# unpause-live/SwiftVideo

Measured on AMD Instinct MI355X. Metric: Gpix/s + achieved HBM GB/s, 1080p NV12→BGRA+scale+4-layer composite, 1/2/4/8 GPU, higher is better.
Workload: dtype f32; 1 GPU; pipeline: 4 x 1080p NV12 -> BGRA (BT.601 int) + bilinear scale to 720p + 4-layer alpha composite, one launch per batch; frames_per_launch_per_gpu=256, kernel=tick_bgra_stream, full=False

## Files before the change

swiftvideo_amd/csrc/chipvideo.cpp:

```cpp
#include "../../include/chipvideo.h"

#include <hip/hip_runtime.h>
#include <hip/hiprtc.h>

#include <algorithm>
#include <atomic>
#include <cctype>
#include <cstdarg>
#include <cmath>
#include <cstdio>
#include <cstring>
#include <map>
#include <memory>
#include <mutex>
#include <string>
#include <vector>

#include "device_types.h"
#include "switches.h"
#include "geom_cache.h"
#include "rebind.h"
#include "lanczos_planar.h"

namespace chv {
const char *bgra_wave_build_flags();
const char *yuv_wave_build_flags();
const char *bgra_stream_build_flags();
const char *yuv_stream_build_flags();
const char *lanczos_build_flags();
hipError_t launch_tick_general(int target_format, const DTick *ticks_host, const DLayer *layers_host, const DTick *ticks, const DLayer *layers,
                               int n_ticks, int maxW, int maxH, hipStream_t stream);
hipError_t launch_selftest(float *out_f, const float *in_f, uint8_t *out_c, const float *num,
                           const float *den, float *out_q, int n, hipStream_t stream);
hipError_t launch_selftest_pack(const int *b, const int *g, const int *r, uint32_t *out, int n, hipStream_t stream);
hipError_t launch_selftest_pack_codes(const float *in, uint32_t *out, int n, hipStream_t stream);
hipError_t launch_selftest_matrices(int dir, int csc, uint32_t *out, uint32_t *mism, hipStream_t stream);
const char *fast_path_name(int path);
bool wave_layers_by_value(int target_format, const DTick *tick_host, const DLayer *layers_host);
bool fast_path_is_wave(int path);
bool fast_path_by_value(int path);
int split_stream_prefix(const DTick *ticks, const DLayer *layers, int n_ticks);
int fast_path_stream_bgra();
int select_tail_path(int target_format, const DTick *ticks, const DLayer *layers, int n_ticks);
int select_fast_path(int target_format, const DTick *ticks, const DLayer *layers, int n_ticks, bool transient = false);
hipError_t launch_tick_fast(int path, const DTick *ticks_host, const DLayer *layers_host,
                            const DTick *ticks, const DLayer *layers, int n_ticks,
                            int maxW, int maxH, hipStream_t stream, GeomCache *tables);
hipError_t launch_snd_s16i(int16_t *out, const int16_t *const *in, int count, int n, const float *gain, const float *fade, hipStream_t stream);
hipError_t launch_me_fullsearch(const DPlane &out, const DPlane &ref, const DPlane &cur, const int32_t *block, const int32_t *window, const int32_t *image,
                                const float *cost256, hipStream_t stream);
hipError_t launch_lanczos(const DPlane &dst, const DPlane &src, const int32_t *fx, const float *wx,
                          int tx, const int32_t *fy, const float *wy, int ty, hipStream_t stream,
                          const DPlane *batch, int n_batch, int stride_x, int first_x, int stride_y);
}

using namespace chv;

static void g_detail_set(const char *msg);

static int parse_switch(const char *name, const char *value, int *out) {
    const std::string n = name ? name : "", v = value ? value : "";
    if (n == "CHV_FORCE_GENERAL") { *out = v == "1" ? 1 : 0; return 0; }
    if (n == "CHV_BGRA_PATH") { *out = v == "wave" ? 1 : v == "tiled" ? 2 : v == "stream" ? 3 : 0; return 1; }
    if (n == "CHV_WAVE_ROWS") { *out = v == "8" ? 8 : v == "16" ? 16 : 0; return 2; }
    if (n == "CHV_TILE_ROWS") { *out = v == "16" ? 16 : v == "32" ? 32 : 0; return 3; }
    if (n == "CHV_SAME_GEOM") { *out = v == "0" ? 0 : 1; return 4; }
    if (n == "CHV_DESC") { *out = v == "host" ? 1 : v == "device" ? 2 : 0; return 5; }
    if (n == "CHV_STREAM") { *out = v == "0" ? 0 : 1; return 6; }
    if (n == "CHV_YUV_STREAM") { *out = v == "0" ? 0 : (v == "force" || v == "2") ? 2 : 1; return 7; }
    if (n == "CHV_WAVE_DMA") { *out = v == "0" ? 0 : 1; return 8; }
    if (n == "CHV_PASS_FUSE") { *out = v == "0" ? 0 : 1; return 9; }
    if (n == "CHV_GEOM_CACHE") { *out = v == "0" ? 0 : v == "eager" ? 2 : 1; return 10; }
    if (n == "CHV_STREAM_ROWS") { const int r = atoi(v.c_str()); *out = (r >= 1 && r <= 4096) ? r : 0; return 11; }
    if (n == "CHV_STREAM_OPAQUE") { *out = v == "0" ? 0 : 1; return 12; }
    if (n == "CHV_REBIND") { *out = v == "scatter" ? 1 : v == "copy" ? 2 : 0; return 13; }
    return -1;
}
static void store_switch(Switches &s, int which, int val) {
    std::atomic<int> *slots[14] = { &s.force_general, &s.bgra_path, &s.wave_rows, &s.tile_rows, &s.same_geom, &s.desc_host, &s.stream, &s.yuv_stream, &s.wave_dma,
                                    &s.pass_fuse, &s.geom_cache, &s.stream_rows, &s.stream_opaque, &s.rebind };
    slots[which]->store(val, std::memory_order_relaxed);
}
Switches &chv::switches() {
    static Switches s;
    static std::once_flag once;
    std::call_once(once, [] {
        static const char *const names[14] = { "CHV_FORCE_GENERAL", "CHV_BGRA_PATH", "CHV_WAVE_ROWS", "CHV_TILE_ROWS", "CHV_SAME_GEOM", "CHV_DESC", "CHV_STREAM", "CHV_YUV_STREAM",
                                               "CHV_WAVE_DMA", "CHV_PASS_FUSE", "CHV_GEOM_CACHE", "CHV_STREAM_ROWS", "CHV_STREAM_OPAQUE", "CHV_REBIND" };
        for (const char *n : names) {
            const char *v = getenv(n);
            int val = 0, which = v ? parse_switch(n, v, &val) : -1;
            if (which >= 0) store_switch(s, which, val);
        }
    });
    return s;
}
static std::atomic<RebindLauncher> g_rebind_launcher{nullptr};
void chv::register_rebind_launcher(RebindLauncher fn) { g_rebind_launcher.store(fn, std::memory_order_release); }
static std::atomic<LanczosPlanarLauncher> g_lanczos_planar_launcher{nullptr};
void chv::register_lanczos_planar_launcher(LanczosPlanarLauncher fn) { g_lanczos_planar_launcher.store(fn, std::memory_order_release); }
DebugCounters &chv::debug_counters() {
    static DebugCounters c;
    return c;
}
extern "C" int chv_debug_set_switch(const char *name, const char *value) {
    int val = 0;
    Switches &s = switches();
    const int which = parse_switch(name, value, &val);
    if (which < 0) { g_detail_set("unknown switch"); return CHV_ERR_INVALID_VALUE; }
    if (!value || !*value) val = (which == 4 || which == 6 || which == 7 || which == 8 || which == 9 || which == 10 || which == 12) ? 1 : 0;
    store_switch(s, which, val);
    return CHV_OK;
}
extern "C" int chv_debug_get_counter(const char *name, unsigned long long *value) {
    static const char *const names[] = { "geom_store_patched", "geom_store_batch_hits", "geom_store_builds", "geom_store_bytes", "geom_store_tables" };
    if (!name || !value) { g_detail_set("null argument"); return CHV_ERR_INVALID_VALUE; }
    for (int i = 0; i < 5; i++)
        if (!strcmp(name, names[i])) { *value = (unsigned long long)geom_store_counter(i); return CHV_OK; }
    if (!strcmp(name, "stream_opaque_launches")) { *value = debug_counters().stream_opaque_launches.load(std::memory_order_relaxed); return CHV_OK; }
    g_detail_set("unknown counter");
    return CHV_ERR_INVALID_VALUE;
}
extern "C" const char *chv_build_flags(void) {
    static const std::string flags = std::string("arch=" CHV_ARCH ";hipcc=" CHV_HIPCC_VERSION ";clang=") + std::to_string(__clang_major__) + "." + std::to_string(__clang_minor__) +
                                     ";fp_contract=off;" + bgra_wave_build_flags() + ";" + yuv_wave_build_flags() + ";" + bgra_stream_build_flags() + ";" +
                                     yuv_stream_build_flags() + ";" + lanczos_build_flags() +
                                     (g_rebind_launcher.load(std::memory_order_acquire) ? ";batch_rebind:scatter=1" : ";batch_rebind:scatter=0");
    return flags.c_str();
}

static thread_local std::string g_detail;
static void g_detail_set(const char *msg) { g_detail = msg; }

static int fail(int code, const char *fmt, ...) __attribute__((format(printf, 2, 3)));
static int fail(int code, const char *fmt, ...) {
    char buf[512];
    va_list ap;
    va_start(ap, fmt);
    vsnprintf(buf, sizeof buf, fmt, ap);
    va_end(ap);
    g_detail = buf;
    return code;
}

static int hip_fail(hipError_t e, const char *what) {
    int code = CHV_ERR_UNKNOWN;
    switch (e) {
    case hipErrorOutOfMemory: code = CHV_ERR_OUT_OF_MEMORY; break;
    case hipErrorInvalidValue: code = CHV_ERR_INVALID_VALUE; break;
    case hipErrorInvalidDevice: code = CHV_ERR_INVALID_DEVICE; break;
    case hipErrorNoDevice: code = CHV_ERR_DEVICE_NOT_AVAILABLE; break;
    case hipErrorInvalidContext: code = CHV_ERR_INVALID_CONTEXT; break;
    case hipErrorNotSupported: code = CHV_ERR_NOT_IMPLEMENTED; break;
    default: break;
    }
    return fail(code, "%s: %s (%d)", what, hipGetErrorString(e), (int)e);
}
#define HIP_TRY(expr)                                         \
    do {                                                      \
        hipError_t _e = (expr);                               \
        if (_e != hipSuccess) return hip_fail(_e, #expr);     \
    } while (0)

extern "C" const char *chv_error_string(int s) {
    switch (s) {
    case CHV_OK: return "success";
    case CHV_ERR_INVALID_VALUE: return "invalidValue";
    case CHV_ERR_OUT_OF_MEMORY: return "outOfMemory";
    case CHV_ERR_INVALID_CONTEXT: return "invalidContext";
    case CHV_ERR_BAD_TARGET: return "badTarget";
    case CHV_ERR_BAD_INPUT: return "badInputData";
    case CHV_ERR_NOT_IMPLEMENTED: return "notImplemented";
    case CHV_ERR_KERNEL_NOT_FOUND: return "computeKernelNotFound";
    case CHV_ERR_DEVICE_NOT_AVAILABLE: return "deviceNotAvailable";
    case CHV_ERR_INVALID_DEVICE: return "invalidDevice";
    case CHV_ERR_INVALID_OPERATION: return "invalidOperation";
    case CHV_ERR_BAD_CONTEXT_STATE: return "badContextState";
    case CHV_ERR_INVALID_PLATFORM: return "invalidPlatform";
    default: return "unknownError";
    }
}
extern "C" const char *chv_last_error_detail(void) { return g_detail.c_str(); }
extern "C" int chv_version(void) { return CHV_VERSION; }

struct KernelName { const char *name; int id; };
static const KernelName kNames[] = {
    { "img_nv12_nv12", CHV_K_IMG_NV12_NV12 },   { "img_bgra_nv12", CHV_K_IMG_BGRA_NV12 },
    { "img_rgba_nv12", CHV_K_IMG_RGBA_NV12 },   { "img_bgra_bgra", CHV_K_IMG_BGRA_BGRA },
    { "img_y420p_y420p", CHV_K_IMG_Y420P_Y420P }, { "img_y420p_nv12", CHV_K_IMG_Y420P_NV12 },
    { "img_clear_nv12", CHV_K_IMG_CLEAR_NV12 }, { "img_clear_yuvs", CHV_K_IMG_CLEAR_YUVS },
    { "img_clear_bgra", CHV_K_IMG_CLEAR_BGRA }, { "img_clear_rgba", CHV_K_IMG_CLEAR_BGRA },
    { "img_rgba_y420p", CHV_K_IMG_RGBA_Y420P }, { "img_bgra_y420p", CHV_K_IMG_BGRA_Y420P },
    { "img_clear_y420p", CHV_K_IMG_CLEAR_Y420P },
    { "img_nv12_bgra", CHV_K_IMG_NV12_BGRA },   { "img_y420p_bgra", CHV_K_IMG_Y420P_BGRA },
    { "img_bgra_bgra_tx", CHV_K_IMG_BGRA_BGRA_TX }, { "img_rgba_bgra_tx", CHV_K_IMG_RGBA_BGRA_TX },
    { "img_rgba_bgra", CHV_K_IMG_RGBA_BGRA_TX },
    { "img_bgra_nv12_int", CHV_K_IMG_BGRA_NV12_INT }, { "img_rgba_nv12_int", CHV_K_IMG_RGBA_NV12_INT },
    { "img_bgra_y420p_int", CHV_K_IMG_BGRA_Y420P_INT }, { "img_rgba_y420p_int", CHV_K_IMG_RGBA_Y420P_INT },
    { "snd_s16i_s16i", CHV_K_SND_S16I_S16I }, { "me_fullsearch", CHV_K_ME_FULLSEARCH },
};

extern "C" int chv_kernel_from_string(const char *name, int *kernel) {
// ... 2058 lines not shown
```

swiftvideo_amd/csrc/kernels_stream.hip.cpp:

```cpp
#include "kernels_stream_body.hip.inc"
#include "stream_select.h"

namespace chv {

hipError_t launch_bgra_stream_opaque(const DTick *ticks_host, const DLayer *layers_host, const DTick *ticks, const DLayer *layers, int n_ticks, bool planar, dim3 grid,
                                     size_t lds, int strips_x, int chunks_y, int rows, hipStream_t stream);

template <int NL, bool PL, bool ABS>
__global__ __launch_bounds__(64 * ST_WAVES, CHV_STREAM_WAVES) void tick_bgra_stream(const DTick *__restrict__ ticks, const DLayer *__restrict__ layers, int n_ticks,
                                                                          int strips_x, int chunks_y, int rows_per_chunk) {
    stream_body<NL, false, PL, ABS>(ticks, layers, n_ticks, strips_x, chunks_y, rows_per_chunk);
}

template <int NL, bool PL, bool ABS>
__global__ __launch_bounds__(64 * ST_WAVES, CHV_STREAM_WAVES) void tick_bgra_stream_one(const StreamOne<NL> a, int strips_x, int chunks_y, int rows_per_chunk) {
    stream_body<NL, true, PL, ABS>(&a.t, a.l, 1, strips_x, chunks_y, rows_per_chunk);
}

static bool stream_plane_ok(const DPlane &p) {
    return (((uintptr_t)p.ptr) & 15) == 0 && (p.pitch & 15) == 0 && ((p.w * p.comps) & 15) == 0 && p.w * p.comps >= 16 && p.h >= 1;
}

#define CHV_STR2(x) #x
#define CHV_STR(x) CHV_STR2(x)
const char *bgra_stream_build_flags() { return "tick_bgra_stream:abl=" CHV_STR(CHV_ST_ABL) ",strips_per_block=" CHV_STR(CHV_STREAM_BLOCK) ",rounds=" CHV_STR(CHV_STREAM_ROUNDS); }

bool bgra_stream_eligible(const DTick *ticks, const DLayer *layers, int n_ticks) {
    if (n_ticks < 1 || !switches().stream.load(std::memory_order_relaxed)) return false;
    const int nl = ticks[0].n_layers;
    if (nl < 1 || nl > 4) return false;
    for (int i = 0; i < n_ticks; i++) {
        const DTick &T = ticks[i];
        if (T.n_layers != nl || !T.clear_first) return false;
        if ((((uintptr_t)T.dst.pl[0].ptr) & 3) != 0 || (T.dst.pl[0].pitch & 3) != 0) return false;
        for (int l = 0; l < nl; l++) {
            const DLayer &Y = layers[T.first_layer + l];
            const int kind0 = layers[ticks[0].first_layer].kind;
            if ((kind0 != LK_BGRA_FROM_NV12 && kind0 != LK_BGRA_FROM_Y420P) || Y.kind != kind0) return false;
            const bool planar = kind0 == LK_BGRA_FROM_Y420P;
            const int need = LF_AXIS_ALIGNED | LF_BOUNDED | LF_NO_FILL | (l ? LF_SAME_GEOM : 0);
            if ((Y.flags & need) != need) return false;
            const float op = Y.u[U_OPACITY];
            if (!(op >= 0.f && op <= 1.f)) return false;
            if (!stream_plane_ok(Y.src.pl[0]) || !stream_plane_ok(Y.src.pl[1])) return false;
            if (Y.src.pl[0].h > 32767 || Y.src.pl[1].h > 16383) return false;
            if (Y.src.pl[1].comps != (planar ? 1 : 2) || Y.src.pl[0].comps != 1) return false;
            if (planar) {
                const DPlane &cu = Y.src.pl[1], &cv = Y.src.pl[2];
                if (!stream_plane_ok(cv) || cv.comps != 1 || cv.w != cu.w || cv.h != cu.h || cv.pitch != cu.pitch) return false;
            }
            if (l == 0) {
                const double kx = 2.0 * (double)Y.u[U_TRANSFORM + 0] * (double)Y.u[U_TEXTURE + 0], ky = 2.0 * (double)Y.u[U_TRANSFORM + 5] * (double)Y.u[U_TEXTURE + 5];
                if (!(kx > 0.0) || !(ky > 0.0)) return false;
                const double sx = kx * Y.src.pl[0].w / (double)T.W;
                if (!(63.0 * sx + 2.0 + 15.0 + 1.0 <= 128.0)) return false;
                if (planar && !(63.0 * (kx * Y.src.pl[1].w / (double)T.W) + 2.0 + 15.0 + 1.0 <= (double)ST_CPP)) return false;
                const double sy = ky * Y.src.pl[0].h / (double)T.H;
                if (!std::isfinite(sy) || sy > 4.0) return false;
            }
        }
    }
    return true;
}

hipError_t launch_bgra_stream(const DTick *ticks_host, const DLayer *layers_host, const DTick *ticks, const DLayer *layers, int n_ticks, int maxW, int maxH, hipStream_t stream) {
    const int nl = ticks_host[0].n_layers;
    const int strips_x = (maxW + 63) / 64;
    const long want = 1024L * CHV_STREAM_WAVES * CHV_STREAM_ROUNDS;
    const long chunks = std::max<long>(1, want / std::max<long>(1, (long)n_ticks * strips_x));
    const long wave_rows = (long)n_ticks * strips_x * maxH;
    const long rows_small = std::min<long>(CHV_STREAM_SMALL_ROWS_MAX, std::max<long>(CHV_STREAM_MIN_ROWS, (wave_rows + CHV_STREAM_SMALL_WAVES - 1) / CHV_STREAM_SMALL_WAVES));
    int rows = (int)std::max<long>(rows_small, (maxH + chunks - 1) / chunks);
    if (CHV_STREAM_ROWS_FIXED > 0) rows = CHV_STREAM_ROWS_FIXED;
    if (const int forced = switches().stream_rows.load(std::memory_order_relaxed)) rows = forced;
    rows = std::max(1, std::min(rows, maxH));
    const int chunks_y = (maxH + rows - 1) / rows;
    const long total = (long)n_ticks * chunks_y * ((strips_x + ST_WAVES - 1) / ST_WAVES);
    dim3 grid((unsigned)(((total + 7) / 8) * 8));
    const bool planar = layers_host[ticks_host[0].first_layer].kind == LK_BGRA_FROM_Y420P;
    const size_t layer_bytes = planar ? (size_t)st_layer_bytes<1, true>() : (size_t)st_layer_bytes<1, false>();
    const size_t lds = (size_t)ST_WAVES * ((size_t)nl * layer_bytes + ST_TAB * (sizeof(uint4) + sizeof(uint32_t)));
    bool absorb = CHV_STREAM_ABSORB != 0;
    for (int i = 0; i < n_ticks && absorb; i++)
        for (int l = 0; l < nl; l++) absorb = absorb && csc_absorbable(layers_host[ticks_host[i].first_layer + l].csc);
    if (absorb && stream_opaque_bottom(ticks_host, layers_host, n_ticks, switches().stream_opaque.load(std::memory_order_relaxed))) {
        const hipError_t err = launch_bgra_stream_opaque(ticks_host, layers_host, ticks, layers, n_ticks, planar, grid, lds, strips_x, chunks_y, rows, stream);
        if (err == hipSuccess) debug_counters().stream_opaque_launches.fetch_add(1, std::memory_order_relaxed);
        return err;
    }
    if (!ticks) {
        if (n_ticks != 1 || !layers_host) return hipErrorInvalidValue;
        auto go = [&](auto tag) {
            constexpr int NL = decltype(tag)::value;
            StreamOne<NL> a;
            a.t = ticks_host[0];
            a.t.first_layer = 0;
            for (int l = 0; l < NL; l++) a.l[l] = layers_host[ticks_host[0].first_layer + l];
            auto fire = [&](auto pl, auto ab) {
                hipLaunchKernelGGL((tick_bgra_stream_one<NL, decltype(pl)::value, decltype(ab)::value>), grid, dim3(64 * ST_WAVES), lds, stream, a, strips_x, chunks_y, rows);
            };
            if (planar) { if (absorb) fire(std::true_type{}, std::true_type{}); else fire(std::true_type{}, std::false_type{}); }
            else { if (absorb) fire(std::false_type{}, std::true_type{}); else fire(std::false_type{}, std::false_type{}); }
        };
        switch (nl) {
        case 1: go(std::integral_constant<int, 1>{}); break;
        case 2: go(std::integral_constant<int, 2>{}); break;
        case 3: go(std::integral_constant<int, 3>{}); break;
        default: go(std::integral_constant<int, 4>{}); break;
        }
        return hipGetLastError();
    }
#define CHV_ST_GO2(N, P, A) hipLaunchKernelGGL((tick_bgra_stream<N, P, A>), grid, dim3(64 * ST_WAVES), lds, stream, ticks, layers, n_ticks, strips_x, chunks_y, rows)
#define CHV_ST_GO(N) do { if (planar) { if (absorb) CHV_ST_GO2(N, true, true); else CHV_ST_GO2(N, true, false); } \
                          else { if (absorb) CHV_ST_GO2(N, false, true); else CHV_ST_GO2(N, false, false); } } while (0)
    switch (nl) {
    case 1: CHV_ST_GO(1); break;
    case 2: CHV_ST_GO(2); break;
    case 3: CHV_ST_GO(3); break;
    default: CHV_ST_GO(4); break;
    }
#undef CHV_ST_GO
#undef CHV_ST_GO2
    return hipGetLastError();
}

}
```

swiftvideo_amd/csrc/kernels_stream_body.hip.inc:

```
#pragma once
#include "wave_common.hip.h"
#include "switches.h"

#include <algorithm>
#include <type_traits>
#include <cmath>

#pragma clang fp contract(off)

namespace chv {

#ifndef CHV_ST_ABL
#define CHV_ST_ABL 0
#endif
#ifndef CHV_STREAM_ABSORB
#define CHV_STREAM_ABSORB 1
#endif
#ifndef CHV_STREAM_PMIX
#define CHV_STREAM_PMIX 1
#endif
#ifndef CHV_STREAM_ROWS_FIXED
#define CHV_STREAM_ROWS_FIXED 0
#endif
#ifndef CHV_STREAM_SMALL_WAVES
#define CHV_STREAM_SMALL_WAVES 4800
#endif
#ifndef CHV_STREAM_SMALL_ROWS_MAX
#define CHV_STREAM_SMALL_ROWS_MAX 12
#endif
#ifndef CHV_STREAM_MIN_ROWS
#define CHV_STREAM_MIN_ROWS 4
#endif
#ifndef CHV_STREAM_ROUNDS
#define CHV_STREAM_ROUNDS 12
#endif
#ifndef CHV_STREAM_WAVES
#define CHV_STREAM_WAVES 6
#endif

constexpr float kRintBias = 8388608.0f;
constexpr int ST_PITCH = 128;
constexpr int ST_YROWS = 8, ST_CROWS = 4;
constexpr int ST_YL = 4 * ST_PITCH, ST_CL = 2 * ST_PITCH;
constexpr int ST_CPP = 96, ST_CLP = 2 * ST_CPP;
template <int NL, bool PL> constexpr int st_layer_bytes() { return ST_PITCH * ST_YROWS + (PL ? 2 * 2 * ST_CLP : ST_PITCH * ST_CROWS); }
constexpr int ST_TAB = 32;
#ifndef CHV_STREAM_BLOCK
#define CHV_STREAM_BLOCK 4
#endif
constexpr int ST_WAVES = CHV_STREAM_BLOCK;


CHV_DEV void st_dma(const uint8_t *p, bool active, uint32_t m0) {
    if (active && !(CHV_ST_ABL & 1))
        asm volatile("s_mov_b32 m0, %0\n\ts_nop 0\n\tglobal_load_lds_dwordx4 %1, off" :: "s"(m0), "v"(p) : "memory");
}

CHV_DEV void st_store(uint8_t *row, uint32_t off, uint32_t v) {
    asm volatile("global_store_dword %0, %1, %2" :: "v"(off), "v"(v), "s"(row) : "memory");
}

struct StTaps { uint32_t y00, y10, y01, y11, u00, u10, u01, u11, v00, v10, v01, v11; };
template <int LO, int LC, int LV>
CHV_DEV void st_taps_read(StTaps &t, uint32_t aY00, uint32_t aY10, uint32_t aY01, uint32_t aY11, uint32_t aC00, uint32_t aC10, uint32_t aC01, uint32_t aC11) {
    asm volatile("ds_read_u8 %0, %12 offset:%20\n\tds_read_u8 %1, %13 offset:%20\n\tds_read_u8 %2, %14 offset:%20\n\tds_read_u8 %3, %15 offset:%20\n\t"
                 "ds_read_u8 %4, %16 offset:%21\n\tds_read_u8 %5, %17 offset:%21\n\tds_read_u8 %6, %18 offset:%21\n\tds_read_u8 %7, %19 offset:%21\n\t"
                 "ds_read_u8 %8, %16 offset:%22\n\tds_read_u8 %9, %17 offset:%22\n\tds_read_u8 %10, %18 offset:%22\n\tds_read_u8 %11, %19 offset:%22"
                 : "=&v"(t.y00), "=&v"(t.y10), "=&v"(t.y01), "=&v"(t.y11), "=&v"(t.u00), "=&v"(t.u10), "=&v"(t.u01), "=&v"(t.u11),
                   "=&v"(t.v00), "=&v"(t.v10), "=&v"(t.v01), "=&v"(t.v11)
                 : "v"(aY00), "v"(aY10), "v"(aY01), "v"(aY11), "v"(aC00), "v"(aC10), "v"(aC01), "v"(aC11), "n"(LO), "n"(LC), "n"(LV));
}
template <int YOUNGER>
CHV_DEV void st_taps_wait(StTaps &t) {
    asm volatile("s_waitcnt lgkmcnt(%12)"
                 : "+v"(t.y00), "+v"(t.y10), "+v"(t.y01), "+v"(t.y11), "+v"(t.u00), "+v"(t.u10), "+v"(t.u01), "+v"(t.u11), "+v"(t.v00), "+v"(t.v10), "+v"(t.v01), "+v"(t.v11)
                 : "n"(YOUNGER));
}

template <int NL, bool ONE, bool PL, bool ABS, bool OPQ = false>
CHV_DEV void stream_body(const DTick *__restrict__ ticks, const DLayer *__restrict__ layers, int n_ticks, int strips_x, int chunks_y, int rows_per_chunk) {
    extern __shared__ __attribute__((aligned(16))) uint8_t lds_all[];
    constexpr int LBYTES = st_layer_bytes<NL, PL>();
    constexpr int CPITCH = PL ? ST_CPP : ST_PITCH, CLB = PL ? ST_CLP : ST_CL;
    constexpr int VOFF = PL ? 2 * NL * ST_CLP : 1;
    constexpr int WBYTES = NL * LBYTES + ST_TAB * (int)(sizeof(uint4) + sizeof(uint32_t));
    const int wave = __builtin_amdgcn_readfirstlane((int)threadIdx.x >> 6);
    uint8_t *lds = lds_all + wave * WBYTES;
    uint4 *rowtab = (uint4 *)(lds + NL * LBYTES);
    uint32_t *rowpos = (uint32_t *)(rowtab + ST_TAB);
    const uint32_t lds0 = (uint32_t)(size_t)lds;
    static_assert(!OPQ || (NL >= 2 && ABS && CHV_STREAM_PMIX), "the opaque-bottom form: two layers or more, absorbed matrices, binary16 blend inputs");
    const int lane = threadIdx.x & 63;
    const int groups_x = (strips_x + ST_WAVES - 1) / ST_WAVES;
    const int total = n_ticks * chunks_y * groups_x;
    const int b = blockIdx.x, per_xcd = (total + 7) >> 3;
    const int idx = (b & 7) * per_xcd + (b >> 3);
    if ((b >> 3) >= per_xcd || idx >= total) return;
    const int tick = idx / (chunks_y * groups_x), rem = idx - tick * (chunks_y * groups_x);
    const int chunk = rem / groups_x, strip = (rem - chunk * groups_x) * ST_WAVES + wave;
    if (strip >= strips_x) return;
    const DTick &T = ticks[ONE ? 0 : tick];
    const DLayer *L = layers + (ONE ? 0 : T.first_layer);
    const int x0 = strip * 64, y0 = chunk * rows_per_chunk;
    if (x0 >= T.W || y0 >= T.H) return;
    const int nrows = min(rows_per_chunk, T.H - y0);
    const DPlane D = T.dst.pl[0];
    const float sx = (float)T.W, sy = (float)T.H;
    const float *U = L[0].u;
    const DPlane SY = L[0].src.pl[0], SC = L[0].src.pl[1];

    const int x = x0 + lane, xe = min(x, T.W - 1);
    const float nx = ((float)xe / sx) * 2.f - 1.f;
    const float t3 = U[U_TRANSFORM + 15];
    const float t0 = nx * U[U_TRANSFORM + 0] + U[U_TRANSFORM + 3];
    const float b0 = nx * U[U_BORDER + 0] + U[U_BORDER + 3];
    const float u = t0 * U[U_TEXTURE + 0] + t3 * U[U_TEXTURE + 3];
    const int cfl = ((b0 >= 0.f && b0 <= 1.f) ? AX_BORDER : 0) | ((t0 >= 0.f && t0 <= 1.f) ? AX_TX : 0) | ((u >= 0.f && u <= 1.f) ? AX_UV : 0);
    int cy, cc;
    float cya, cca;
    lin_axis_raw(u, SY.w, cy, cya); lin_axis_raw(u, SC.w, cc, cca);
    const int cy_first = __builtin_amdgcn_readfirstlane(cy), cc_first = __builtin_amdgcn_readfirstlane(cc);
    const int ycol0 = min(max(cy_first, 0), SY.w - 1) & ~15;
    constexpr int BPC = PL ? 1 : 2;
    const int ccol0 = (min(max(cc_first, 0), SC.w - 1) * BPC) & ~15;
    const int oy0 = min(max(min(max(cy, 0), SY.w - 1) - ycol0, 0), ST_PITCH - 1), oy1 = min(max(min(max(cy + 1, 0), SY.w - 1) - ycol0, 0), ST_PITCH - 1);
    const int oc0 = min(max(min(max(cc, 0), SC.w - 1) * BPC - ccol0, 0), CPITCH - BPC), oc1 = min(max(min(max(cc + 1, 0), SC.w - 1) * BPC - ccol0, 0), CPITCH - BPC);
    int oc0v = oc0, oc1v = oc1;
    asm("" : "+v"(oc0v), "+v"(oc1v));
    const float iya = (1.0f - cya) * kTapScale, ya = cya * kTapScale, ica = (1.0f - cca) * kTapScale, ca = cca * kTapScale;
    const bool lane_pic = cfl == AX_ALL && x < T.W;
    const int nvecY = (__builtin_amdgcn_readlane(oy1, 63) >> 4) + 1, nvecC = ((__builtin_amdgcn_readlane(oc1, 63) + BPC - 1) >> 4) + 1;

    std::conditional_t<ABS, CscAbsorbed, CscFolded> csc[NL];
    float al[NL], ial[NL], nrb[NL], al24[NL];
    float ial24 = 0.f;
    const uint8_t *planeY[NL], *planeC[NL], *planeV[NL];
#pragma unroll
    for (int l = 0; l < NL; l++) {
        if constexpr (ABS) csc[l] = csc_fold_absorbed(L[l].csc);
        else csc[l] = csc_fold_biased(kCsc[L[l].csc & 3]);
        al[l] = 1.0f * L[l].u[U_OPACITY]; ial[l] = 1.f - al[l];
        al24[l] = al[l] * kTapScale;
        nrb[l] = -kRintBias * ial[l];
        if (!(OPQ && l <= 1)) asm volatile("" : "+v"(nrb[l]));
        if (OPQ && l == 1) ial24 = ial[1] * kTapScale;
        planeY[l] = L[l].src.pl[0].ptr; planeC[l] = L[l].src.pl[1].ptr; planeV[l] = L[l].src.pl[PL ? 2 : 1].ptr;
    }
    const int liC = PL ? (lane * 43) >> 9 : lane >> 4, inC = PL ? lane - liC * 12 : lane & 15;
    static_assert(((63 * 43) >> 9) == 5 && ((47 * 43) >> 9) == 3 && ((48 * 43) >> 9) == 4 && ((11 * 43) >> 9) == 0 && ((12 * 43) >> 9) == 1, "lane / 12");
    const int rrY = (lane >> 3) & 3, rrC = PL ? (inC >= 6 ? 1 : 0) : (lane >> 3) & 1, vecC = PL ? inC - 6 * rrC : lane & 7;
    const int colY = min(ycol0 + 16 * (lane & 7), SY.w - 16), colC = min(ccol0 + 16 * vecC, SC.w * BPC - 16);

    int lastY, lastC;
    {
        const int ye = min(y0 + nrows - 1, T.H - 1);
        const float ny = ((float)ye / sy) * 2.f - 1.f;
        const float t1 = ny * U[U_TRANSFORM + 5] + U[U_TRANSFORM + 7];
        const float v = t1 * U[U_TEXTURE + 5] + t3 * U[U_TEXTURE + 7];
        int ry, rc;
        float a_;
        lin_axis_raw(v, SY.h, ry, a_); lin_axis_raw(v, SC.h, rc, a_);
        lastY = __builtin_amdgcn_readfirstlane(ry) + 1; lastC = __builtin_amdgcn_readfirstlane(rc) + 1;
    }
    uint32_t pending = 0u;
    uint32_t alpha_word = 0xFF000000u;
    asm volatile("" : "+v"(alpha_word));
    int issued = 0, seqY = 0, seqC = 0;
    int nextY = 0, nextC = 0, landY = 0, landC = 0, baseY = 0, baseC = 0;
    for (int j = 0; j < nrows; j++) {
        if ((j & (ST_TAB - 1)) == 0) {
            wave_lds_fence();
            const int ye = min(y0 + j + min(lane, ST_TAB - 1), T.H - 1);
            const float ny = ((float)ye / sy) * 2.f - 1.f;
            const float t1 = ny * U[U_TRANSFORM + 5] + U[U_TRANSFORM + 7];
            const float b1 = ny * U[U_BORDER + 5] + U[U_BORDER + 7];
            const float v = t1 * U[U_TEXTURE + 5] + t3 * U[U_TEXTURE + 7];
            const int rfl = ((b1 >= 0.f && b1 <= 1.f) ? AX_BORDER : 0) | ((t1 >= 0.f && t1 <= 1.f) ? AX_TX : 0) | ((v >= 0.f && v <= 1.f) ? AX_UV : 0);
            int ry, rc;
            float rya, rca;
            lin_axis_raw(v, SY.h, ry, rya); lin_axis_raw(v, SC.h, rc, rca);
            if (lane < ST_TAB) {
                rowtab[lane] = make_uint4(__float_as_uint(rya), __float_as_uint(rca), __float_as_uint(1.0f - rya), __float_as_uint(1.0f - rca));
                rowpos[lane] = ((uint32_t)min(max(ry, -32768), 32767) & 0xFFFFu) | (((uint32_t)min(max(rc, -16384), 16383) & 0x7FFFu) << 16) | (rfl == AX_ALL ? 0x80000000u : 0u);
            }
            wave_lds_fence();
        }
        const uint4 re = rowtab[j & (ST_TAB - 1)];
        const int rp = __builtin_amdgcn_readfirstlane((int)rowpos[j & (ST_TAB - 1)]);
        const int ry = (int)((uint32_t)rp << 16) >> 16, rc = (int)((uint32_t)rp << 1) >> 17;
        const bool row_pic = rp < 0;
        const float yb = __uint_as_float(re.x), cbw = __uint_as_float(re.y);
        if (j == 0) {
            baseY = ry; baseC = rc; nextY = ry; nextC = rc; landY = ry; landC = rc;
        }
        {
            auto await = [&](int younger) {
                if (younger <= 0) asm volatile("s_waitcnt vmcnt(0)" ::: "memory");
                else if (younger == 1) asm volatile("s_waitcnt vmcnt(1)" ::: "memory");
                else if (younger == 2) asm volatile("s_waitcnt vmcnt(2)" ::: "memory");
                else asm volatile("s_waitcnt vmcnt(3)" ::: "memory");
                wave_lds_fence();
            };
            const bool needY = ry + 1 >= landY, needC = rc + 1 >= landC;
            const bool wantY = ry + ST_YROWS / 2 >= nextY && nextY <= lastY, wantC = rc + ST_CROWS / 2 >= nextC && nextC <= lastC;
            if (needY | needC | wantY | wantC) {
            if (needY) { await(issued - seqY); landY = nextY; }
            if (needC) { await(issued - seqC); landC = nextC; }
            if (wantY || wantC) asm volatile("s_waitcnt lgkmcnt(0)" ::: "memory");
            while (ry + ST_YROWS / 2 >= nextY && nextY <= lastY) {
                const uint32_t slot = (uint32_t)((((nextY - baseY) >> 2) & 1) * (NL * ST_YL));
                const int r = min(max(nextY + rrY, 0), SY.h - 1);
                const size_t roff = (size_t)r * SY.pitch + (size_t)colY;
#pragma unroll
                for (int l0 = 0; l0 < NL; l0 += 2) {
                    const uint8_t *pa = planeY[l0], *pb = planeY[l0 + 1 < NL ? l0 + 1 : l0];
                    st_dma((lane < 32 ? pa : pb) + roff, (lane < 32 || l0 + 1 < NL) && (lane & 7) < nvecY && nextY + rrY <= lastY, lds0 + slot + (uint32_t)(l0 * ST_YL));
                }
                nextY += 4; issued += (NL + 1) / 2; seqY = issued;
            }
            while (rc + ST_CROWS / 2 >= nextC && nextC <= lastC) {
                const uint32_t slot = (uint32_t)(2 * NL * ST_YL + (((nextC - baseC) >> 1) & 1) * (NL * CLB));
                const int r = min(max(nextC + rrC, 0), SC.h - 1);
                const size_t roff = (size_t)r * SC.pitch + (size_t)colC;
                const int li = liC;
                const bool act = li < NL && vecC < nvecC && nextC + rrC <= lastC;
                const uint8_t *pl = li == 0 ? planeC[0] : li == 1 ? planeC[NL > 1 ? 1 : 0] : li == 2 ? planeC[NL > 2 ? 2 : 0] : planeC[NL > 3 ? 3 : 0];
                st_dma(pl + roff, act, lds0 + slot);
                if constexpr (PL) {
                    const uint8_t *pv = li == 0 ? planeV[0] : li == 1 ? planeV[NL > 1 ? 1 : 0] : li == 2 ? planeV[NL > 2 ? 2 : 0] : planeV[NL > 3 ? 3 : 0];
                    st_dma(pv + roff, act, lds0 + slot + (uint32_t)(2 * NL * ST_CLP));
                    issued += 1;
                }
                nextC += 2; issued += 1; seqC = issued;
            }
            if (ry + 1 >= landY || rc + 1 >= landC) { await(0); landY = nextY; landC = nextC; }
            }
        }
        if (j > 0 && x < T.W && !(CHV_ST_ABL & 2)) st_store(D.ptr + (size_t)(y0 + j - 1) * D.pitch, (uint32_t)x * 4u, pending);
        auto yoff = [&](int q) { return ((q >> 2) & 1) * (NL * ST_YL) + (q & 3) * ST_PITCH; };
        auto coff = [&](int q) { return 2 * NL * ST_YL + ((q >> 1) & 1) * (NL * CLB) + (q & 1) * CPITCH; };
        const int sY0 = yoff(ry - baseY), sY1 = yoff(ry + 1 - baseY), sC0 = coff(rc - baseC), sC1 = coff(rc + 1 - baseC);
        const uint32_t bY0 = lds0 + (uint32_t)sY0, bY1 = lds0 + (uint32_t)sY1, bC0 = lds0 + (uint32_t)sC0, bC1 = lds0 + (uint32_t)sC1;
        const uint32_t aY00 = bY0 + (uint32_t)oy0, aY10 = bY0 + (uint32_t)oy1, aY01 = bY1 + (uint32_t)oy0, aY11 = bY1 + (uint32_t)oy1;
        const uint32_t aC00 = bC0 + (uint32_t)oc0v, aC10 = bC0 + (uint32_t)oc1v, aC01 = bC1 + (uint32_t)oc0v, aC11 = bC1 + (uint32_t)oc1v;
        const float iyb = __uint_as_float(re.z), icb = __uint_as_float(re.w);
        const float w00 = iya * iyb, w10 = ya * iyb, w01 = iya * yb, w11 = ya * yb;
        const float c00 = ica * icb, c10 = ca * icb, c01 = ica * cbw, c11 = ca * cbw;
        float r0 = 0.f, r1 = 0.f, r2 = 0.f;
        [[maybe_unused]] int32_t q0 = 0, q1 = 0, q2 = 0;
        constexpr bool AHEAD = !PL;
        StTaps taps[2];
        auto read_layer = [&](auto lt) {
            constexpr int l = decltype(lt)::value;
            st_taps_read<l * ST_YL, l * CLB, l * CLB + VOFF>(taps[l & 1], aY00, aY10, aY01, aY11, aC00, aC10, aC01, aC11);
        };
        if (!(CHV_ST_ABL & 4)) read_layer(std::integral_constant<int, 0>{});
        auto layer = [&](auto lt) {
            constexpr int l = decltype(lt)::value;
            if constexpr (l < NL && !(CHV_ST_ABL & 4)) {
            if constexpr (l + 1 < NL && AHEAD) { read_layer(std::integral_constant<int, l + 1>{}); st_taps_wait<12>(taps[l & 1]); }
            else {
                if constexpr (l > 0 && !AHEAD) read_layer(lt);
                st_taps_wait<0>(taps[l & 1]);
            }
            const StTaps &t = taps[l & 1];
            const float fy = cs_mix_h(w00, w10, w01, w11, tap_h(t.y00), tap_h(t.y10), tap_h(t.y01), tap_h(t.y11));
            const float fu = cs_mix_h(c00, c10, c01, c11, tap_h(t.u00), tap_h(t.u10), tap_h(t.u01), tap_h(t.u11));
            const float fv = cs_mix_h(c00, c10, c01, c11, tap_h(t.v00), tap_h(t.v10), tap_h(t.v01), tap_h(t.v11));
            if constexpr (ABS && CHV_STREAM_PMIX) {
                int32_t cb, cg, cr;
                yuv_to_bgr_fixed_absorbed(csc[l], fy, fu, fv, cb, cg, cr);
                const float a24 = al24[l];
                if constexpr (OPQ && l == 0) {
                    q0 = cb; q1 = cg; q2 = cr;
                    return;
                } else if constexpr (OPQ && l == 1) {
                    r0 = __builtin_fmaf(a24, (float)code_h(cb), __builtin_fmaf(ial24, (float)code_h(q0), 0.0f));
                    r1 = __builtin_fmaf(a24, (float)code_h(cg), __builtin_fmaf(ial24, (float)code_h(q1), 0.0f));
                    r2 = __builtin_fmaf(a24, (float)code_h(cr), __builtin_fmaf(ial24, (float)code_h(q2), 0.0f));
                } else if (l == 0) {
                    r0 = __builtin_fmaf(a24, (float)code_h(cb), 0.0f); r1 = __builtin_fmaf(a24, (float)code_h(cg), 0.0f); r2 = __builtin_fmaf(a24, (float)code_h(cr), 0.0f);
                } else {
                    r0 = __builtin_fmaf(a24, (float)code_h(cb), __builtin_fmaf(r0, ial[l], nrb[l]));
                    r1 = __builtin_fmaf(a24, (float)code_h(cg), __builtin_fmaf(r1, ial[l], nrb[l]));
                    r2 = __builtin_fmaf(a24, (float)code_h(cr), __builtin_fmaf(r2, ial[l], nrb[l]));
                }
                if (l + 1 < NL) { r0 += kRintBias; r1 += kRintBias; r2 += kRintBias; }
                return;
            }
            float pb, pg, pr;
            if constexpr (ABS) yuv_to_bgr_floats_absorbed(csc[l], fy, fu, fv, pb, pg, pr);
            else yuv_to_bgr_floats(csc[l], (int)code_biased(fy), (int)code_biased(fu), (int)code_biased(fv), pb, pg, pr);
            if (l == 0) {
                r0 = pb * al[0]; r1 = pg * al[0]; r2 = pr * al[0];
            } else {
                r0 = __builtin_fmaf(pb, al[l], __builtin_fmaf(r0, ial[l], nrb[l]));
                r1 = __builtin_fmaf(pg, al[l], __builtin_fmaf(r1, ial[l], nrb[l]));
                r2 = __builtin_fmaf(pr, al[l], __builtin_fmaf(r2, ial[l], nrb[l]));
            }
            if (l + 1 < NL) { r0 += kRintBias; r1 += kRintBias; r2 += kRintBias; }
            }
        };
        layer(std::integral_constant<int, 0>{}); layer(std::integral_constant<int, 1>{}); layer(std::integral_constant<int, 2>{}); layer(std::integral_constant<int, 3>{});
        uint32_t out;
        asm("v_cvt_pk_u8_f32 %0, %1, 0, %2" : "=v"(out) : "v"(r0), "v"(alpha_word));
        asm("v_cvt_pk_u8_f32 %0, %1, 1, %0" : "+v"(out) : "v"(r1));
        asm("v_cvt_pk_u8_f32 %0, %1, 2, %0" : "+v"(out) : "v"(r2));
        const uint32_t res = (lane_pic && row_pic) ? out : alpha_word;
        pending = res;
    }
    if (nrows > 0 && x < T.W && !(CHV_ST_ABL & 2)) st_store(D.ptr + (size_t)(y0 + nrows - 1) * D.pitch, (uint32_t)x * 4u, pending);
}

template <int NL>
struct StreamOne {
    DTick t;
    DLayer l[NL];
};

}
```

swiftvideo_amd/csrc/kernels_stream_opq.hip.cpp:

```cpp
#include "kernels_stream_body.hip.inc"

namespace chv {

template <int NL, bool PL, bool ABS>
__global__ __launch_bounds__(64 * ST_WAVES, CHV_STREAM_WAVES) void tick_bgra_stream_ob(const DTick *__restrict__ ticks, const DLayer *__restrict__ layers, int n_ticks,
                                                                             int strips_x, int chunks_y, int rows_per_chunk) {
    stream_body<NL, false, PL, ABS, true>(ticks, layers, n_ticks, strips_x, chunks_y, rows_per_chunk);
}

template <int NL, bool PL, bool ABS>
__global__ __launch_bounds__(64 * ST_WAVES, CHV_STREAM_WAVES) void tick_bgra_stream_ob_one(const StreamOne<NL> a, int strips_x, int chunks_y, int rows_per_chunk) {
    stream_body<NL, true, PL, ABS, true>(&a.t, a.l, 1, strips_x, chunks_y, rows_per_chunk);
}

hipError_t launch_bgra_stream_opaque(const DTick *ticks_host, const DLayer *layers_host, const DTick *ticks, const DLayer *layers, int n_ticks, bool planar, dim3 grid,
                                     size_t lds, int strips_x, int chunks_y, int rows, hipStream_t stream) {
    const int nl = ticks_host[0].n_layers;
    if (nl < 2 || nl > 4) return hipErrorInvalidValue;
    auto go = [&](auto tag, auto pl) {
        constexpr int NL = decltype(tag)::value;
        constexpr bool PL = decltype(pl)::value;
        if (!ticks) {
            StreamOne<NL> a;
            a.t = ticks_host[0];
            a.t.first_layer = 0;
            for (int l = 0; l < NL; l++) a.l[l] = layers_host[ticks_host[0].first_layer + l];
            hipLaunchKernelGGL((tick_bgra_stream_ob_one<NL, PL, true>), grid, dim3(64 * ST_WAVES), lds, stream, a, strips_x, chunks_y, rows);
        } else {
            hipLaunchKernelGGL((tick_bgra_stream_ob<NL, PL, true>), grid, dim3(64 * ST_WAVES), lds, stream, ticks, layers, n_ticks, strips_x, chunks_y, rows);
        }
    };
    auto layers_of = [&](auto pl) {
        switch (nl) {
        case 2: go(std::integral_constant<int, 2>{}, pl); break;
        case 3: go(std::integral_constant<int, 3>{}, pl); break;
        default: go(std::integral_constant<int, 4>{}, pl); break;
        }
    };
    if (!ticks && (n_ticks != 1 || !layers_host)) return hipErrorInvalidValue;
    if (planar) layers_of(std::true_type{}); else layers_of(std::false_type{});
    return hipGetLastError();
}

}
```

swiftvideo_amd/csrc/stream_select.h:

```cpp
#pragma once
#include "device_types.h"

#include <string.h>

namespace chv {

inline bool stream_opaque_bottom(const DTick *ticks_host, const DLayer *layers_host, int n_ticks, int enabled) {
    if (!enabled || n_ticks < 1) return false;
    const float one = 1.0f;
    for (int i = 0; i < n_ticks; i++) {
        if (ticks_host[i].n_layers < 2) return false;
        if (memcmp(&layers_host[ticks_host[i].first_layer].u[U_OPACITY], &one, sizeof one) != 0) return false;
    }
    return true;
}

}
```

swiftvideo_amd/csrc/switches.h:

```cpp
#pragma once
#include <atomic>

namespace chv {

struct Switches {
    std::atomic<int> force_general{0};
    std::atomic<int> bgra_path{0};
    std::atomic<int> wave_rows{0};
    std::atomic<int> tile_rows{0};
    std::atomic<int> same_geom{1};
    std::atomic<int> desc_host{0};
    std::atomic<int> stream{1};
    std::atomic<int> yuv_stream{1};
    std::atomic<int> wave_dma{1};
    std::atomic<int> geom_cache{1};
    std::atomic<int> pass_fuse{1};
    std::atomic<int> stream_rows{0};
    std::atomic<int> stream_opaque{1};
    std::atomic<int> rebind{0};
};
Switches &switches();

struct DebugCounters {
    std::atomic<unsigned long long> stream_opaque_launches{0};
};
DebugCounters &debug_counters();

}
```

Measured before the change: 204.4 Gpix/s.

## Carry chroma row taps in registers across output rows in opaque stream kernel

Adds a chroma-carry variant of the opaque-bottom NV12 stream kernel. It keeps the two chroma source rows' U/V taps for every layer in registers and reloads them from LDS only when the source chroma row changes. Luma reads are double-buffered per layer with explicit lgkmcnt waits. The goal is fewer LDS reads and less wait latency when vertical chroma scaling is at most 1. In exchange it adds register pressure, lowers the launch-bound occupancy hint to 5 waves, and adds an optional minimum-LDS knob.

```diff
diff --git a/swiftvideo_amd/csrc/chipvideo.cpp b/swiftvideo_amd/csrc/chipvideo.cpp
--- a/swiftvideo_amd/csrc/chipvideo.cpp
+++ b/swiftvideo_amd/csrc/chipvideo.cpp
@@ -73,20 +73,21 @@
     if (n == "CHV_GEOM_CACHE") { *out = v == "0" ? 0 : v == "eager" ? 2 : 1; return 10; }
     if (n == "CHV_STREAM_ROWS") { const int r = atoi(v.c_str()); *out = (r >= 1 && r <= 4096) ? r : 0; return 11; }
     if (n == "CHV_STREAM_OPAQUE") { *out = v == "0" ? 0 : 1; return 12; }
+    if (n == "CHV_STREAM_CARRY") { *out = v == "0" ? 0 : 1; return 14; }
     if (n == "CHV_REBIND") { *out = v == "scatter" ? 1 : v == "copy" ? 2 : 0; return 13; }
     return -1;
 }
 static void store_switch(Switches &s, int which, int val) {
-    std::atomic<int> *slots[14] = { &s.force_general, &s.bgra_path, &s.wave_rows, &s.tile_rows, &s.same_geom, &s.desc_host, &s.stream, &s.yuv_stream, &s.wave_dma,
-                                    &s.pass_fuse, &s.geom_cache, &s.stream_rows, &s.stream_opaque, &s.rebind };
+    std::atomic<int> *slots[15] = { &s.force_general, &s.bgra_path, &s.wave_rows, &s.tile_rows, &s.same_geom, &s.desc_host, &s.stream, &s.yuv_stream, &s.wave_dma,
+                                    &s.pass_fuse, &s.geom_cache, &s.stream_rows, &s.stream_opaque, &s.rebind, &s.stream_carry };
     slots[which]->store(val, std::memory_order_relaxed);
 }
 Switches &chv::switches() {
     static Switches s;
     static std::once_flag once;
     std::call_once(once, [] {
-        static const char *const names[14] = { "CHV_FORCE_GENERAL", "CHV_BGRA_PATH", "CHV_WAVE_ROWS", "CHV_TILE_ROWS", "CHV_SAME_GEOM", "CHV_DESC", "CHV_STREAM", "CHV_YUV_STREAM",
-                                               "CHV_WAVE_DMA", "CHV_PASS_FUSE", "CHV_GEOM_CACHE", "CHV_STREAM_ROWS", "CHV_STREAM_OPAQUE", "CHV_REBIND" };
+        static const char *const names[15] = { "CHV_FORCE_GENERAL", "CHV_BGRA_PATH", "CHV_WAVE_ROWS", "CHV_TILE_ROWS", "CHV_SAME_GEOM", "CHV_DESC", "CHV_STREAM", "CHV_YUV_STREAM",
+                                               "CHV_WAVE_DMA", "CHV_PASS_FUSE", "CHV_GEOM_CACHE", "CHV_STREAM_ROWS", "CHV_STREAM_OPAQUE", "CHV_REBIND", "CHV_STREAM_CARRY" };
         for (const char *n : names) {
             const char *v = getenv(n);
             int val = 0, which = v ? parse_switch(n, v, &val) : -1;
@@ -108,7 +109,7 @@
     Switches &s = switches();
     const int which = parse_switch(name, value, &val);
     if (which < 0) { g_detail_set("unknown switch"); return CHV_ERR_INVALID_VALUE; }
-    if (!value || !*value) val = (which == 4 || which == 6 || which == 7 || which == 8 || which == 9 || which == 10 || which == 12) ? 1 : 0;
+    if (!value || !*value) val = (which == 4 || which == 6 || which == 7 || which == 8 || which == 9 || which == 10 || which == 12 || which == 14) ? 1 : 0;
     store_switch(s, which, val);
     return CHV_OK;
 }
@@ -118,6 +119,7 @@
     for (int i = 0; i < 5; i++)
         if (!strcmp(name, names[i])) { *value = (unsigned long long)geom_store_counter(i); return CHV_OK; }
     if (!strcmp(name, "stream_opaque_launches")) { *value = debug_counters().stream_opaque_launches.load(std::memory_order_relaxed); return CHV_OK; }
+    if (!strcmp(name, "stream_carry_launches")) { *value = debug_counters().stream_carry_launches.load(std::memory_order_relaxed); return CHV_OK; }
     g_detail_set("unknown counter");
     return CHV_ERR_INVALID_VALUE;
 }
diff --git a/swiftvideo_amd/csrc/kernels_stream.hip.cpp b/swiftvideo_amd/csrc/kernels_stream.hip.cpp
--- a/swiftvideo_amd/csrc/kernels_stream.hip.cpp
+++ b/swiftvideo_amd/csrc/kernels_stream.hip.cpp
@@ -79,7 +79,8 @@
     dim3 grid((unsigned)(((total + 7) / 8) * 8));
     const bool planar = layers_host[ticks_host[0].first_layer].kind == LK_BGRA_FROM_Y420P;
     const size_t layer_bytes = planar ? (size_t)st_layer_bytes<1, true>() : (size_t)st_layer_bytes<1, false>();
-    const size_t lds = (size_t)ST_WAVES * ((size_t)nl * layer_bytes + ST_TAB * (sizeof(uint4) + sizeof(uint32_t)));
+    size_t lds = (size_t)ST_WAVES * ((size_t)nl * layer_bytes + ST_TAB * (sizeof(uint4) + sizeof(uint32_t)));
+    if (CHV_STREAM_LDS_MIN > 0) lds = std::max<size_t>(lds, CHV_STREAM_LDS_MIN);
     bool absorb = CHV_STREAM_ABSORB != 0;
     for (int i = 0; i < n_ticks && absorb; i++)
         for (int l = 0; l < nl; l++) absorb = absorb && csc_absorbable(layers_host[ticks_host[i].first_layer + l].csc);
diff --git a/swiftvideo_amd/csrc/kernels_stream_body.hip.inc b/swiftvideo_amd/csrc/kernels_stream_body.hip.inc
--- a/swiftvideo_amd/csrc/kernels_stream_body.hip.inc
+++ b/swiftvideo_amd/csrc/kernels_stream_body.hip.inc
@@ -36,6 +36,9 @@
 #endif
 #ifndef CHV_STREAM_WAVES
 #define CHV_STREAM_WAVES 6
+#endif
+#ifndef CHV_STREAM_LDS_MIN
+#define CHV_STREAM_LDS_MIN 0
 #endif
 
 constexpr float kRintBias = 8388608.0f;
@@ -77,7 +80,49 @@
                  : "n"(YOUNGER));
 }
 
-template <int NL, bool ONE, bool PL, bool ABS, bool OPQ = false>
+template <int NL> struct StCarry { uint32_t c[NL][4]; };
+static_assert(ST_CL == 256, "the offsets of st_carry_read");
+#define CHV_ST_CARRY_LAYER(L, OU, OV) "ds_read_u8 %[c" #L "0], %[a0] offset:" #OU "\n\tds_read_u8 %[c" #L "1], %[a1] offset:" #OU "\n\t" \
+                                      "ds_read_u8 %[c" #L "2], %[a0] offset:" #OV "\n\tds_read_u8 %[c" #L "3], %[a1] offset:" #OV "\n\t"
+#define CHV_ST_CARRY_REGS(S, L, C) [c##L##0] C((S).c[L][0]), [c##L##1] C((S).c[L][1]), [c##L##2] C((S).c[L][2]), [c##L##3] C((S).c[L][3])
+template <int NL>
+CHV_DEV void st_carry_read(StCarry<NL> &s, uint32_t a0, uint32_t a1) {
+    static_assert(NL >= 2 && NL <= 4, "the carry form: two to four layers");
+    if constexpr (NL == 2)
+        asm volatile(CHV_ST_CARRY_LAYER(0, 0, 1) CHV_ST_CARRY_LAYER(1, 256, 257)
+                     : CHV_ST_CARRY_REGS(s, 0, "+v"), CHV_ST_CARRY_REGS(s, 1, "+v") : [a0] "v"(a0), [a1] "v"(a1));
+    else if constexpr (NL == 3)
+        asm volatile(CHV_ST_CARRY_LAYER(0, 0, 1) CHV_ST_CARRY_LAYER(1, 256, 257) CHV_ST_CARRY_LAYER(2, 512, 513)
+                     : CHV_ST_CARRY_REGS(s, 0, "+v"), CHV_ST_CARRY_REGS(s, 1, "+v"), CHV_ST_CARRY_REGS(s, 2, "+v") : [a0] "v"(a0), [a1] "v"(a1));
+    else
+        asm volatile(CHV_ST_CARRY_LAYER(0, 0, 1) CHV_ST_CARRY_LAYER(1, 256, 257) CHV_ST_CARRY_LAYER(2, 512, 513) CHV_ST_CARRY_LAYER(3, 768, 769)
+                     : CHV_ST_CARRY_REGS(s, 0, "+v"), CHV_ST_CARRY_REGS(s, 1, "+v"), CHV_ST_CARRY_REGS(s, 2, "+v"), CHV_ST_CARRY_REGS(s, 3, "+v")
+                     : [a0] "v"(a0), [a1] "v"(a1));
+}
+template <int NL>
+CHV_DEV void st_carry_tie(StCarry<NL> &s) {
+    if constexpr (NL == 2) asm volatile("" : CHV_ST_CARRY_REGS(s, 0, "+v"), CHV_ST_CARRY_REGS(s, 1, "+v"));
+    else if constexpr (NL == 3) asm volatile("" : CHV_ST_CARRY_REGS(s, 0, "+v"), CHV_ST_CARRY_REGS(s, 1, "+v"), CHV_ST_CARRY_REGS(s, 2, "+v"));
+    else asm volatile("" : CHV_ST_CARRY_REGS(s, 0, "+v"), CHV_ST_CARRY_REGS(s, 1, "+v"), CHV_ST_CARRY_REGS(s, 2, "+v"), CHV_ST_CARRY_REGS(s, 3, "+v"));
+}
+struct StLuma { uint32_t y00, y10, y01, y11; };
+template <int LO>
+CHV_DEV void st_luma_read(StLuma &t, uint32_t aY00, uint32_t aY10, uint32_t aY01, uint32_t aY11) {
+    asm volatile("ds_read_u8 %0, %4 offset:%8\n\tds_read_u8 %1, %5 offset:%8\n\tds_read_u8 %2, %6 offset:%8\n\tds_read_u8 %3, %7 offset:%8"
+                 : "=&v"(t.y00), "=&v"(t.y10), "=&v"(t.y01), "=&v"(t.y11) : "v"(aY00), "v"(aY10), "v"(aY01), "v"(aY11), "n"(LO));
+}
+template <int YOUNGER>
+CHV_DEV void st_luma_wait(StLuma &t) {
+    asm volatile("s_waitcnt lgkmcnt(%4)" : "+v"(t.y00), "+v"(t.y10), "+v"(t.y01), "+v"(t.y11) : "n"(YOUNGER));
+}
+template <int NL, int YOUNGER>
+CHV_DEV void st_carry_wait(StLuma &t, StCarry<NL> &even, StCarry<NL> &odd) {
+    st_luma_wait<YOUNGER>(t);
+    st_carry_tie<NL>(even);
+    st_carry_tie<NL>(odd);
+}
+
+template <int NL, bool ONE, bool PL, bool ABS, bool OPQ = false, bool CRY = false>
 CHV_DEV void stream_body(const DTick *__restrict__ ticks, const DLayer *__restrict__ layers, int n_ticks, int strips_x, int chunks_y, int rows_per_chunk) {
     extern __shared__ __attribute__((aligned(16))) uint8_t lds_all[];
     constexpr int LBYTES = st_layer_bytes<NL, PL>();
@@ -90,6 +135,7 @@
     uint32_t *rowpos = (uint32_t *)(rowtab + ST_TAB);
     const uint32_t lds0 = (uint32_t)(size_t)lds;
     static_assert(!OPQ || (NL >= 2 && ABS && CHV_STREAM_PMIX), "the opaque-bottom form: two layers or more, absorbed matrices, binary16 blend inputs");
+    static_assert(!CRY || (OPQ && !PL && !ONE && !(CHV_ST_ABL & 4)), "the chroma-carry form: opaque-bottom batch kernels of NV12 sources");
     const int lane = threadIdx.x & 63;
     const int groups_x = (strips_x + ST_WAVES - 1) / ST_WAVES;
     const int total = n_ticks * chunks_y * groups_x;
@@ -167,6 +213,8 @@
     asm volatile("" : "+v"(alpha_word));
     int issued = 0, seqY = 0, seqC = 0;
     int nextY = 0, nextC = 0, landY = 0, landC = 0, baseY = 0, baseC = 0;
+    [[maybe_unused]] StCarry<CRY ? NL : 2> cset[2] = {};
+    [[maybe_unused]] int held0 = 0x40000000, held1 = 0x40000000;
     for (int j = 0; j < nrows; j++) {
         if ((j & (ST_TAB - 1)) == 0) {
             wave_lds_fence();
@@ -248,6 +296,64 @@
         const float c00 = ica * icb, c10 = ca * icb, c01 = ica * cbw, c11 = ca * cbw;
         float r0 = 0.f, r1 = 0.f, r2 = 0.f;
         [[maybe_unused]] int32_t q0 = 0, q1 = 0, q2 = 0;
+        if constexpr (CRY) {
+            asm volatile("" :: "v"(w00), "v"(w10), "v"(w01), "v"(w11), "v"(c00), "v"(c10), "v"(c01), "v"(c11));
+            const int par = (rc - baseC) & 1;
+            const int row0 = rc + par, row1 = rc + 1 - par;
+            if (held0 != row0) {
+                const uint32_t bc = lds0 + (uint32_t)coff(row0 - baseC);
+                st_carry_read<NL>(cset[0], bc + (uint32_t)oc0v, bc + (uint32_t)oc1v);
+                held0 = row0;
+            }
+            if (held1 != row1) {
+                const uint32_t bc = lds0 + (uint32_t)coff(row1 - baseC);
+                st_carry_read<NL>(cset[1], bc + (uint32_t)oc0v, bc + (uint32_t)oc1v);
+                held1 = row1;
+            }
+            StLuma lum[2];
+            st_luma_read<0>(lum[0], aY00, aY10, aY01, aY11);
+            st_carry_wait<NL, 0>(lum[0], cset[0], cset[1]);
+            auto rest = [&](auto top_even) {
+                constexpr int TOP = decltype(top_even)::value ? 0 : 1;
+                auto clayer = [&](auto lt) {
+                    constexpr int l = decltype(lt)::value;
+                    if constexpr (l < NL) {
+                        if constexpr (l + 1 < NL) st_luma_read<(l + 1) * ST_YL>(lum[(l + 1) & 1], aY00, aY10, aY01, aY11);
+                        if constexpr (l >= 1 && l + 1 < NL) st_luma_wait<4>(lum[l & 1]);
+                        else if constexpr (l >= 1) st_luma_wait<0>(lum[l & 1]);
+                        const StLuma &t = lum[l & 1];
+                        const uint32_t *ct = cset[TOP].c[l], *cb_ = cset[1 - TOP].c[l];
+                        const float fy = cs_mix_h(w00, w10, w01, w11, tap_h(t.y00), tap_h(t.y10), tap_h(t.y01), tap_h(t.y11));
+                        const float fu = cs_mix_h(c00, c10, c01, c11, tap_h(ct[0]), tap_h(ct[1]), tap_h(cb_[0]), tap_h(cb_[1]));
+                        const float fv = cs_mix_h(c00, c10, c01, c11, tap_h(ct[2]), tap_h(ct[3]), tap_h(cb_[2]), tap_h(cb_[3]));
+                        int32_t cb, cg, cr;
+                        yuv_to_bgr_fixed_absorbed(csc[l], fy, fu, fv, cb, cg, cr);
+                        const float a24 = al24[l];
+                        if constexpr (l == 0) {
+                            q0 = cb; q1 = cg; q2 = cr;
+                            return;
+                        } else if constexpr (l == 1) {
+                            r0 = __builtin_fmaf(a24, (float)code_h(cb), __builtin_fmaf(ial24, (float)code_h(q0), 0.0f));
+                            r1 = __builtin_fmaf(a24, (float)code_h(cg), __builtin_fmaf(ial24, (float)code_h(q1), 0.0f));
+                            r2 = __builtin_fmaf(a24, (float)code_h(cr), __builtin_fmaf(ial24, (float)code_h(q2), 0.0f));
+                        } else {
+                            r0 = __builtin_fmaf(a24, (float)code_h(cb), __builtin_fmaf(r0, ial[l], nrb[l]));
+                            r1 = __builtin_fmaf(a24, (float)code_h(cg), __builtin_fmaf(r1, ial[l], nrb[l]));
+                            r2 = __builtin_fmaf(a24, (float)code_h(cr), __builtin_fmaf(r2, ial[l], nrb[l]));
+                        }
+                        if (l + 1 < NL) { r0 += kRintBias; r1 += kRintBias; r2 += kRintBias; }
+                    }
+                };
+                clayer(std::integral_constant<int, 0>{}); clayer(std::integral_constant<int, 1>{}); clayer(std::integral_constant<int, 2>{}); clayer(std::integral_constant<int, 3>{});
+                uint32_t out;
+                asm("v_cvt_pk_u8_f32 %0, %1, 0, %2" : "=v"(out) : "v"(r0), "v"(alpha_word));
+                asm("v_cvt_pk_u8_f32 %0, %1, 1, %0" : "+v"(out) : "v"(r1));
+                asm("v_cvt_pk_u8_f32 %0, %1, 2, %0" : "+v"(out) : "v"(r2));
+                pending = (lane_pic && row_pic) ? out : alpha_word;
+            };
+            if (par) rest(std::false_type{}); else rest(std::true_type{});
+            continue;
+        }
         constexpr bool AHEAD = !PL;
         StTaps taps[2];
         auto read_layer = [&](auto lt) {
diff --git a/swiftvideo_amd/csrc/kernels_stream_carry.hip.cpp b/swiftvideo_amd/csrc/kernels_stream_carry.hip.cpp
--- /dev/null
+++ b/swiftvideo_amd/csrc/kernels_stream_carry.hip.cpp
@@ -0,0 +1,27 @@
+#include "kernels_stream_body.hip.inc"
+
+namespace chv {
+
+#ifndef CHV_STREAM_CARRY_WAVES
+#define CHV_STREAM_CARRY_WAVES 5
+#endif
+
+template <int NL>
+__global__ __launch_bounds__(64 * ST_WAVES, CHV_STREAM_CARRY_WAVES) void tick_bgra_stream_cc(const DTick *__restrict__ ticks, const DLayer *__restrict__ layers, int n_ticks,
+                                                                                   int strips_x, int chunks_y, int rows_per_chunk) {
+    stream_body<NL, false, false, true, true, true>(ticks, layers, n_ticks, strips_x, chunks_y, rows_per_chunk);
+}
+
+hipError_t launch_bgra_stream_carry(int nl, const DTick *ticks, const DLayer *layers, int n_ticks, dim3 grid, size_t lds, int strips_x, int chunks_y, int rows,
+                                    hipStream_t stream) {
+    if (!ticks || !layers) return hipErrorInvalidValue;
+    switch (nl) {
+    case 2: hipLaunchKernelGGL((tick_bgra_stream_cc<2>), grid, dim3(64 * ST_WAVES), lds, stream, ticks, layers, n_ticks, strips_x, chunks_y, rows); break;
+    case 3: hipLaunchKernelGGL((tick_bgra_stream_cc<3>), grid, dim3(64 * ST_WAVES), lds, stream, ticks, layers, n_ticks, strips_x, chunks_y, rows); break;
+    case 4: hipLaunchKernelGGL((tick_bgra_stream_cc<4>), grid, dim3(64 * ST_WAVES), lds, stream, ticks, layers, n_ticks, strips_x, chunks_y, rows); break;
+    default: return hipErrorInvalidValue;
+    }
+    return hipGetLastError();
+}
+
+}
diff --git a/swiftvideo_amd/csrc/kernels_stream_opq.hip.cpp b/swiftvideo_amd/csrc/kernels_stream_opq.hip.cpp
--- a/swiftvideo_amd/csrc/kernels_stream_opq.hip.cpp
+++ b/swiftvideo_amd/csrc/kernels_stream_opq.hip.cpp
@@ -1,6 +1,10 @@
 #include "kernels_stream_body.hip.inc"
+#include "stream_select.h"
 
 namespace chv {
+
+hipError_t launch_bgra_stream_carry(int nl, const DTick *ticks, const DLayer *layers, int n_ticks, dim3 grid, size_t lds, int strips_x, int chunks_y, int rows,
+                                    hipStream_t stream);
 
 template <int NL, bool PL, bool ABS>
 __global__ __launch_bounds__(64 * ST_WAVES, CHV_STREAM_WAVES) void tick_bgra_stream_ob(const DTick *__restrict__ ticks, const DLayer *__restrict__ layers, int n_ticks,
@@ -17,6 +21,11 @@
                                      size_t lds, int strips_x, int chunks_y, int rows, hipStream_t stream) {
     const int nl = ticks_host[0].n_layers;
     if (nl < 2 || nl > 4) return hipErrorInvalidValue;
+    if (stream_chroma_carry(ticks_host, layers_host, n_ticks, planar, !ticks, switches().stream_carry.load(std::memory_order_relaxed))) {
+        const hipError_t err = launch_bgra_stream_carry(nl, ticks, layers, n_ticks, grid, lds, strips_x, chunks_y, rows, stream);
+        if (err == hipSuccess) debug_counters().stream_carry_launches.fetch_add(1, std::memory_order_relaxed);
+        return err;
+    }
     auto go = [&](auto tag, auto pl) {
         constexpr int NL = decltype(tag)::value;
         constexpr bool PL = decltype(pl)::value;
diff --git a/swiftvideo_amd/csrc/stream_select.h b/swiftvideo_amd/csrc/stream_select.h
--- a/swiftvideo_amd/csrc/stream_select.h
+++ b/swiftvideo_amd/csrc/stream_select.h
@@ -15,4 +15,17 @@
     return true;
 }
 
+inline bool stream_chroma_carry(const DTick *ticks_host, const DLayer *layers_host, int n_ticks, bool planar, bool by_value, int enabled) {
+    if (!enabled || planar || by_value || n_ticks < 1) return false;
+    for (int i = 0; i < n_ticks; i++) {
+        const DTick &T = ticks_host[i];
+        if (T.n_layers < 2 || T.n_layers > 4 || T.H < 1) return false;
+        const DLayer &Y = layers_host[T.first_layer];
+        const double ky = 2.0 * (double)Y.u[U_TRANSFORM + 5] * (double)Y.u[U_TEXTURE + 5];
+        const double sc = ky * Y.src.pl[1].h / (double)T.H;
+        if (!(sc > 0.0) || !(sc <= 1.0)) return false;
+    }
+    return true;
 }
+
+}
diff --git a/swiftvideo_amd/csrc/switches.h b/swiftvideo_amd/csrc/switches.h
--- a/swiftvideo_amd/csrc/switches.h
+++ b/swiftvideo_amd/csrc/switches.h
@@ -17,12 +17,14 @@
     std::atomic<int> pass_fuse{1};
     std::atomic<int> stream_rows{0};
     std::atomic<int> stream_opaque{1};
+    std::atomic<int> stream_carry{1};
     std::atomic<int> rebind{0};
 };
 Switches &switches();
 
 struct DebugCounters {
     std::atomic<unsigned long long> stream_opaque_launches{0};
+    std::atomic<unsigned long long> stream_carry_launches{0};
 };
 DebugCounters &debug_counters();
 
```

Result: faster. 215.2 Gpix/s, median of 6 (+5.2%).
